# intel/hdk

Measured on AMD Instinct MI355X. Metric: rows/sec, 1B-row int64 GROUP BY SUM, higher is better.
Workload: dtype int64; 1 GPU; C2: SELECT key, SUM(val) GROUP BY key; int64, 64 uniform keys; rows=1000000000, rows_per_gpu=1000000000, fragments=32, fragments_per_gpu=32, fragment_rows=32000000, layout=perfect hash, keyless, 64 entries, parallelism=fragment f -> GPU f mod 1; one GPU

## Files before the change

hdk_amd/csrc/scan_bhm.hip:

```cpp
#include <string.h>

#include <algorithm>

#include "host_match.h"
#include "scan_bhm.h"
#include "scan_bhm_part.h"
#include "scan_bhm_host.h"
#include "scan_bhm_shapes.h"

namespace hdk {

constexpr uint32_t kBhmMaxLdsBytes = 144u << 10;
constexpr uint32_t kBhmSmallLdsBytes = 40u << 10;
constexpr uint32_t kBhmReplicatedBytes = 32u << 10;
constexpr int64_t kBhmMaxAbsVal = (1ll << 19) - 1;
static bool bhm_off() { return hdk_sw(SW_NO_BHM) != nullptr || hdk_sw(SW_NO_BH_LDS) != nullptr || hdk_sw(SW_NO_BH_DENSE) != nullptr; }

static uint32_t bits_for(uint64_t codes) {
  uint32_t b = 1;
  while ((1ull << b) < codes) ++b;
  return b;
}

struct BhmGeom {
// ... 269 lines not shown
      sw.packed = der.packed;
    } else if (sw.kind == BMW_NN) {
      if (!src.nullable) {
        sw.kind = BMW_ROWS;
        sw.packed = a->rows_packed;
      } else if (der.packed >= 0) {
        sw.packed = der.packed;
      } else {
        from_field(der.has_mx != 0);
      }
    } else {
      from_field(sw.kind == BMW_MAX);
    }
  }
  *per_entry_out = 8u * static_cast<uint32_t>(a->npacked) + static_cast<uint32_t>(a->mm_bytes) + (a->rows_packed < 0 ? 4u : 0u);
  *amax_out = amax;
  g->nk = a->nkeys;
  g->ns = a->nsrc;
  return true;
}

static uint64_t bhm_lds_layout(BhmArgs* a, uint32_t per_entry) {
  a->e1 = (a->entries + 1 + 1) & ~1u;
  a->off_mm = 8u * static_cast<uint32_t>(a->npacked) * a->e1;
  a->off_rows = a->off_mm + static_cast<uint32_t>(a->mm_bytes) * a->e1;
  return static_cast<uint64_t>(a->e1) * per_entry;
}

static bool match_bhm(const hdk_hip_plan* p, const hdk_hip_kernel_options* ko, BhmArgs* a, BhmGeom* g) {
  uint32_t per_entry;
  int64_t amax;
  if (!match_bhm_shape(p, ko, a, g, &per_entry, &amax)) return false;
  const uint64_t one = bhm_lds_layout(a, per_entry);
  if (one > kBhmMaxLdsBytes) return false;
  uint32_t rep_bytes = (static_cast<uint32_t>(one) + 15u) & ~15u;
  uint32_t rep = 16;
  while (rep > 1 && static_cast<uint64_t>(rep_bytes + 16) * rep > kBhmReplicatedBytes) rep >>= 1;
  if (rep > 1) {
    while (rep_bytes % 256 != 16) rep_bytes += 16;
  }
  a->rep = rep;
  a->rep_bytes = rep_bytes;
  a->lds_bytes = rep_bytes * rep;
  g->block = a->lds_bytes > kBhmSmallLdsBytes ? 1024 : 256;
  g->grid_per_cu = g->block == 1024 ? 1 : 3;
  const int64_t by_sum = ((1ll << 39) - 1) / amax;
  a->max_rows_per_block = static_cast<uint32_t>(std::min<int64_t>(by_sum, 1ll << 23));
  return true;
}

constexpr uint32_t kBhmPartLdsBytes = 50u << 10;
struct BhmPartLayout {
  size_t cursor_bytes, tuple_bytes, slab_bytes, total;
};
static bool match_bhm_part(const hdk_hip_plan* p, const hdk_hip_kernel_options* ko, BhmPartArgs* pg, BhmGeom* g, BhmPartLayout* l) {
  if (hdk_sw(SW_NO_BHM_PARTITIONS) || hdk_sw(SW_NO_BH_PARTITIONS)) return false;
  memset(pg, 0, sizeof(*pg));
  BhmArgs* a = &pg->b;
  uint32_t per_entry;
  int64_t amax;
  if (!match_bhm_shape(p, ko, a, g, &per_entry, &amax)) return false;
  const bool always = hdk_sw(SW_BH_PARTITIONS_ALWAYS) != nullptr;
  if (!always && ko->total_rows < (4ull << 20)) return false;
  const uint32_t total = a->entries;
  uint32_t w = 4;
  while (w < 14 && (static_cast<uint64_t>((2u << w) + 2) * per_entry) <= kBhmPartLdsBytes) ++w;
  uint32_t min_bins = 128;
  if (const char* e = hdk_sw(SW_BHM_PART_MIN_BINS)) min_bins = static_cast<uint32_t>(std::max(1, atoi(e)));
  while (w > 4 && ((total + (1u << w) - 1) >> w) < min_bins) --w;
  while (((total + (1u << w) - 1) >> w) > kPbMaxBins) ++w;
  if (static_cast<uint64_t>((1u << w) + 2) * per_entry > kBhmPartLdsBytes) return false;
  pg->w = w;
  pg->nbins = (total + (1u << w) - 1) >> w;
  pg->total_entries = total;
  uint32_t pos = w;
  for (int s = 0; s < a->nsrc; ++s) {
    const uint32_t cb = bits_for(static_cast<uint64_t>(a->src[s].raw_span) + 2);
    if (pos + cb > 32) return false;
    pg->cshift[s] = pos;
    pg->cmask[s] = static_cast<uint32_t>((1ull << cb) - 1);
    pos += cb;
  }
  pg->tw = (pos <= 16 && !hdk_sw(SW_BHM_WIDE_TUPLES)) ? 2 : 4;
  a->entries = 1u << w;
  const uint64_t one = bhm_lds_layout(a, per_entry);
  uint32_t prep_bytes = (static_cast<uint32_t>(one) + 15u) & ~15u;
  uint32_t prep = 1;
  if (const char* e = hdk_sw(SW_BHM_PART_REPLICAS)) prep = static_cast<uint32_t>(std::max(1, atoi(e)));
  while (prep > 1 && static_cast<uint64_t>(prep_bytes + 16) * prep > kBhmReplicatedBytes) prep >>= 1;
  if (prep > 1) {
    while (prep_bytes % 256 != 16) prep_bytes += 16;
  }
  a->rep = prep;
  a->rep_bytes = prep_bytes;
  a->lds_bytes = prep_bytes * prep;
  a->max_rows_per_block = 0xFFFFFFFFu;
  const int64_t by_sum = ((1ll << 39) - 1) / amax;
  uint64_t generation = static_cast<uint64_t>(std::min<int64_t>(by_sum, 1ll << 23)) & ~4095ull;
  if (const char* e = hdk_sw(SW_BHM_PART_GENERATION)) generation = static_cast<uint64_t>(std::max(1, atoi(e))) * 4096;
  if (generation < 4096) return false;
  pg->generation = static_cast<uint32_t>(generation);
  for (int w = 0; w < a->wpe; ++w) pg->wop[w] = g->wop[w];
  pg->cap_limit = 0xFFFFFFF0ull;
  pg->parts = 64;
  const uint64_t avg = ko->total_rows / (static_cast<uint64_t>(pg->nbins) * kPbXcds) + 1;
  pg->part_tuples = static_cast<uint32_t>(std::min<uint64_t>((std::max<uint64_t>(2 * avg, 65536) + 4095) & ~4095ull, 1u << 30));
  if (const char* e = hdk_sw(SW_BHM_PART_TUPLES)) pg->part_tuples = static_cast<uint32_t>(std::max(1, atoi(e))) * 4096u;
  pg->total_rows = ko->total_rows;
  pg->region_max = ((ko->total_rows / kPbXcds) * 5 / 2 + static_cast<uint64_t>(pg->nbins) * 4104 + 7) & ~7ull;
  if (pg->region_max > 0xFFFFFFF0ull) return false;
  pg->sample_stride = static_cast<uint32_t>(std::min<uint64_t>(std::max<uint64_t>(ko->total_rows / (256ull * (16 / g->width)) / 1536, 1), 1u << 16));
  if (const char* e = hdk_sw(SW_BHM_PART_SAMPLE_STRIDE)) pg->sample_stride = static_cast<uint32_t>(std::max(1, atoi(e)));
  l->cursor_bytes = static_cast<size_t>(pg->nbins) * kPbXcds * kPbCursorStride * sizeof(uint32_t) + kBlWords * sizeof(uint32_t);
  l->cursor_bytes = (l->cursor_bytes + 255) & ~static_cast<size_t>(255);
  l->tuple_bytes = std::max((static_cast<size_t>(kPbXcds) * pg->region_max + kBhmPartBlock * 16) * pg->tw, static_cast<size_t>(total) * a->wpe * 8);
  l->tuple_bytes = (l->tuple_bytes + 255) & ~static_cast<size_t>(255);
  l->slab_bytes = static_cast<size_t>(kPbXcds) * total * a->wpe * 8;
  if (l->slab_bytes > (1ull << 30)) return false;
  l->total = 256 + l->cursor_bytes + l->tuple_bytes + l->slab_bytes;
  return true;
}

HDK_BHM_DEFINE_KERNELS(4, false, HDK_BHM_SHAPE_FN_NULLS, HDK_BHM_PLAIN_BODY_YES)

struct BhmStaticShape {
  int nk, ns;
  uint32_t code[kBhmMaxDer];
  const void* (*aggregate)(int tw, bool nulls);
};
#define HDK_BHM_SHAPE_ROW(NK, NS, D0, D1, D2, D3)                                                                            \
  {NK, NS, {D0, D1, D2, D3}, [](int tw, bool nulls) -> const void* {                                                         \
     if (nulls) {                                                                                                            \
       return tw == 2 ? reinterpret_cast<const void*>(hdk_bhm_aggregate<BhmStatic<D0, D1, D2, D3, true>, NS, 2>)             \
                      : reinterpret_cast<const void*>(hdk_bhm_aggregate<BhmStatic<D0, D1, D2, D3, true>, NS, 4>);            \
     }                                                                                                                       \
     return tw == 2 ? reinterpret_cast<const void*>(hdk_bhm_aggregate<BhmStatic<D0, D1, D2, D3, false>, NS, 2>)              \
                    : reinterpret_cast<const void*>(hdk_bhm_aggregate<BhmStatic<D0, D1, D2, D3, false>, NS, 4>);             \
   }},
static const BhmStaticShape kBhmShapes[] = {HDK_BHM_SHAPES(HDK_BHM_SHAPE_ROW)};
#undef HDK_BHM_SHAPE_ROW
constexpr int kBhmNumShapes = static_cast<int>(sizeof(kBhmShapes) / sizeof(kBhmShapes[0]));

template <class F4, class F4Q, class F8, class F8Q>
static const void* bhm_by_quarter(const BhmArgs& a, const BhmGeom& g, F4 f4, F4Q f4q, F8 f8, F8Q f8q) {
  return g.width == 8 ? (a.nquals ? f8q() : f8()) : (a.nquals ? f4q() : f4());
}
static const void* bhm_scatter_kernel(const BhmArgs& a, const BhmGeom& g) {
  return bhm_by_quarter(
      a, g, [&] { return BhmKernels<4, false>::scatter(g.nk, g.ns); }, [&] { return BhmKernels<4, true>::scatter(g.nk, g.ns); },
      [&] { return BhmKernels<8, false>::scatter(g.nk, g.ns); }, [&] { return BhmKernels<8, true>::scatter(g.nk, g.ns); });
}

template <int W>
static const void* bhm_sample_kernel_w(int nk) {
  return nk == 1 ? reinterpret_cast<const void*>(hdk_bhm_part_sample<1, W>)
                 : (nk == 2 ? reinterpret_cast<const void*>(hdk_bhm_part_sample<2, W>) : reinterpret_cast<const void*>(hdk_bhm_part_sample<3, W>));
}
static const void* bhm_sample_kernel(const BhmGeom& g) { return g.width == 8 ? bhm_sample_kernel_w<8>(g.nk) : bhm_sample_kernel_w<4>(g.nk); }

static uint32_t bhm_plain_flags(const BhmArgs& a);
static void bhm_shift_to_codes(BhmArgs* a) {
  a->plain_flags = bhm_plain_flags(*a);
  for (int d = 0; d < a->nder; ++d) {
    BhmDer& der = a->der[d];
    const BhmSrc& src = a->src[der.src];
    if (der.mul == 1) {
// ... 75 lines not shown
      if (same) return sh.aggregate(tw, a.any_nullable != 0);
    }
  }
  if (bhm_plain_flags(a) && !hdk_sw(SW_BHM_DYNAMIC)) {
    return tw == 2 ? bhm_aggregate_plain<2>(g.ns) : bhm_aggregate_plain<4>(g.ns);
  }
  return tw == 2 ? bhm_aggregate_dynamic<2>(g.ns) : bhm_aggregate_dynamic<4>(g.ns);
}

const char* bhm_kernel_name(const hdk_hip_plan* p, const hdk_hip_kernel_options* ko) {
  BhmArgs a;
  BhmGeom g;
  if (!match_bhm(p, ko, &a, &g)) {
    BhmPartArgs pg;
    BhmPartLayout l;
    if (match_bhm_part(p, ko, &pg, &g, &l)) {
      return g.perfect ? "hdk_bhm_scatter,hdk_bhm_aggregate,hdk_bhm_reduce_slabs,hdk_finalize"
                       : "hdk_bhm_scatter,hdk_bhm_aggregate,hdk_bhm_reduce_slabs,hdk_bhm_fold";
    }
    return nullptr;
  }
  return g.perfect ? "hdk_scan_agg_bhm,hdk_bhm_reduce_slabs,hdk_finalize" : "hdk_scan_agg_bhm,hdk_bhm_reduce_slabs,hdk_bhm_fold";
}

static int32_t launch_bhm_folds(const hdk_hip_plan* plan, const hdk_hip_plan* d_plan, const KernParams& kp, const hdk_hip_kernel_options* ko,
                                const hdk_hip_device_properties* props, hipStream_t s, const BhmArgs& a, const BhmGeom& g, uint32_t entries,
                                const int64_t* fold_slabs, uint32_t fold_count) {
  int32_t st;
  if (g.perfect) {
    st = launch_finalize_slabs(d_plan, fold_slabs, kp.groupby_buf, fold_count, plan->entry_count, a.flag, s);
    if (st) return st;
  } else {
    BhmFoldArgs f;
    memset(&f, 0, sizeof(f));
    f.plan = d_plan;
    f.kp = kp;
    f.slabs = fold_slabs;
    f.flag = a.flag;
    f.num_slabs = fold_count;
    f.entries = entries;
    f.out_entry_count = plan->entry_count;
    f.wpe = a.wpe;
    for (int w = 0; w < a.wpe; ++w) f.wop[w] = g.wop[w];
    f.nword_mask = g.nword_mask;
    f.key_form = a.key_form;
    f.key_lo = g.key_lo;
    f.null_entry = g.null_entry;
    f.key_null_word = a.key_null_word;
    if (fold_count <= 16 && entries >= 2048) {
      hipLaunchKernelGGL(hdk_bhm_fold<1>, dim3((entries + 255) / 256), dim3(256), 0, s, f);
    } else {
      hipLaunchKernelGGL(hdk_bhm_fold<0>, dim3((entries + 3) / 4), dim3(256), 0, s, f);
    }
    HDK_HIP_CHECK(hipGetLastError());
  }
  if (hdk_sw(SW_BHM_FLAG_IS_ERROR)) {
    hipLaunchKernelGGL(hdk_bhm_flag_is_error<0>, dim3(1), dim3(1), 0, s, a.flag, kp.error_code);
    HDK_HIP_CHECK(hipGetLastError());
    return HDK_HIP_OK;
  }
  return launch_scan_global_armed(plan, d_plan, kp, ko, props, s, a.flag);
}

static int32_t launch_bhm_part(const hdk_hip_plan* plan, const hdk_hip_plan* d_plan, const KernParams& kp, const hdk_hip_kernel_options* ko,
                               const hdk_hip_device_properties* props, hipStream_t s, BhmPartArgs& pg, const BhmGeom& g, const BhmPartLayout& l,
                               bool* launched) {
  AsyncScratch scratch(s);
  if (hipMallocAsync(&scratch.p, l.total, s) != hipSuccess) {
    (void)hipGetLastError();
    scratch.p = nullptr;
    return HDK_HIP_OK;
  }
  int8_t* base = static_cast<int8_t*>(scratch.p);
  HDK_HIP_CHECK(hipMemsetAsync(base, 0, 256 + l.cursor_bytes, s));
  BhmArgs& a = pg.b;
  a.plan = d_plan;
  a.kp = kp;
  a.flag = reinterpret_cast<uint32_t*>(base);
  pg.fill = reinterpret_cast<uint32_t*>(base + 256);
  pg.layout = pg.fill + static_cast<size_t>(pg.nbins) * kPbXcds * kPbCursorStride;
  pg.tuples = reinterpret_cast<uint32_t*>(base + 256 + l.cursor_bytes);
  a.slabs = reinterpret_cast<int64_t*>(base + 256 + l.cursor_bytes + l.tuple_bytes);
  const void* sk = bhm_scatter_kernel(a, g);
  const size_t scatter_lds = bhm_scatter_lds(g.width);
  HDK_HIP_CHECK(hipFuncSetAttribute(sk, hipFuncAttributeMaxDynamicSharedMemorySize, static_cast<int>(scatter_lds)));
  const unsigned g1 = scatter_grid(sk, kBhmPartBlock, scatter_lds, props, kBhmPartWaves * 256 / kBhmPartBlock);
  void* kargs[] = {&pg};
  const uint64_t sampled_tiles = ko->total_rows / (256ull * (16 / g.width)) / pg.sample_stride + 1;
  const unsigned g0 = static_cast<unsigned>(std::min<uint64_t>((sampled_tiles + 3) / 4, static_cast<uint64_t>(props->num_cu)));
  HDK_HIP_CHECK(hipLaunchKernel(bhm_sample_kernel(g), dim3(g0), dim3(256), kargs, 0, s));
  HDK_HIP_CHECK(hipLaunchKernel(reinterpret_cast<const void*>(hdk_bhm_part_layout<0>), dim3(1), dim3(kPbMaxBins), kargs, 0, s));
  HDK_HIP_CHECK(hipLaunchKernel(sk, dim3(g1), dim3(kBhmPartBlock), kargs, scatter_lds, s));
  const void* ak = bhm_aggregate_kernel(a, g, static_cast<int>(pg.tw));
  BhmPartArgs pgb = pg;
  bhm_shift_to_codes(&pgb.b);
  void* kargs_b[] = {&pgb};
  if (a.lds_bytes > (48u << 10)) {
    HDK_HIP_CHECK(hipFuncSetAttribute(ak, hipFuncAttributeMaxDynamicSharedMemorySize, static_cast<int>(a.lds_bytes)));
  }
  {
    BhmSlabInitArgs ia;
    memset(&ia, 0, sizeof(ia));
    ia.slabs = a.slabs;
    ia.words = static_cast<uint64_t>(kPbXcds) * pg.total_entries * static_cast<uint32_t>(a.wpe);
    ia.wpe = a.wpe;
    for (int w = 0; w < a.wpe; ++w) ia.wop[w] = g.wop[w];
    const unsigned gi = static_cast<unsigned>(std::min<uint64_t>((ia.words + 255) / 256, static_cast<uint64_t>(props->num_cu) * 8));
    hipLaunchKernelGGL(hdk_bhm_slab_init<0>, dim3(gi), dim3(256), 0, s, ia);
    HDK_HIP_CHECK(hipGetLastError());
  }
  HDK_HIP_CHECK(hipLaunchKernel(ak, dim3(pg.nbins * kPbXcds, pg.parts), dim3(kBhmAggBlock), kargs_b, a.lds_bytes, s));
  BhmReduceArgs r;
  memset(&r, 0, sizeof(r));
  r.in = a.slabs;
  r.out = reinterpret_cast<int64_t*>(base + 256 + l.cursor_bytes);
  r.flag = a.flag;
  r.num_slabs = kPbXcds;
  r.groups = 1;
  r.words = pg.total_entries * static_cast<uint32_t>(a.wpe);
  r.wpe = a.wpe;
  for (int w = 0; w < a.wpe; ++w) r.wop[w] = g.wop[w];
  hipLaunchKernelGGL(hdk_bhm_reduce_slabs<0>, dim3((r.words + 255) / 256, 1), dim3(256), 0, s, r);
  HDK_HIP_CHECK(hipGetLastError());
  const int32_t st = launch_bhm_folds(plan, d_plan, kp, ko, props, s, a, g, pg.total_entries, r.out, 1);
  if (st) return st;
  *launched = true;
  return HDK_HIP_OK;
}

int32_t launch_bhm(const hdk_hip_plan* plan, const hdk_hip_plan* d_plan, const KernParams& kp, const hdk_hip_kernel_options* ko,
                   const hdk_hip_device_properties* props, hipStream_t s, bool* launched) {
  *launched = false;
  BhmArgs a;
  BhmGeom g;
  if (!match_bhm(plan, ko, &a, &g)) {
    BhmPartArgs pg;
    BhmPartLayout l;
    if (match_bhm_part(plan, ko, &pg, &g, &l)) return launch_bhm_part(plan, d_plan, kp, ko, props, s, pg, g, l, launched);
    return HDK_HIP_OK;
  }
  bool is_static;
  const void* k = bhm_kernel(a, g, &is_static);
  if (a.lds_bytes > (48u << 10)) {
    HDK_HIP_CHECK(hipFuncSetAttribute(k, hipFuncAttributeMaxDynamicSharedMemorySize, static_cast<int>(a.lds_bytes)));
  }
  const uint32_t cu = static_cast<uint32_t>(props->num_cu);
  uint32_t grid = std::min(resident_grid(k, g.block, a.lds_bytes, props), g.grid_per_cu * cu);
  if (const char* e = hdk_sw(SW_BHM_BLOCKS_PER_CU)) grid = std::max(1, atoi(e)) * cu;
  constexpr uint64_t kTileRows256 = 256ull * 4 * kBhmU;
  const uint64_t tile_rows = kTileRows256 * (g.block / 256);
  const uint64_t budget = a.max_rows_per_block > 4 * tile_rows ? a.max_rows_per_block - 4 * tile_rows : tile_rows;
  const uint64_t need = (2 * ko->total_rows + budget - 1) / budget;
  if (need > grid) grid = static_cast<uint32_t>(std::min<uint64_t>(need, 1u << 16));
  if (ko->grid_dim_x) grid = ko->grid_dim_x;
  const uint32_t words = a.entries * static_cast<uint32_t>(a.wpe);
  const uint32_t red_groups = grid > 16 ? 4u : 0u;
  const size_t slab_bytes = (static_cast<size_t>(grid) * words * 8 + 255) & ~static_cast<size_t>(255);
  const size_t red_bytes = static_cast<size_t>(red_groups) * words * 8;
  AsyncScratch scratch(s);
  if (hipMallocAsync(&scratch.p, 256 + slab_bytes + red_bytes, s) != hipSuccess) {
    (void)hipGetLastError();
    scratch.p = nullptr;
    return HDK_HIP_OK;
  }
  HDK_HIP_CHECK(hipMemsetAsync(scratch.p, 0, 256, s));
  a.plan = d_plan;
  a.kp = kp;
// ... 31 lines not shown
```

hdk_amd/csrc/scan_bhm_part.h:

```cpp
#pragma once
#include "scan_bhm.h"
#include "part_scatter_batch.h"

namespace hdk {

#ifndef HDK_BHM_PART_BLOCK
#define HDK_BHM_PART_BLOCK 512
#endif
constexpr int kBhmPartBlock = HDK_BHM_PART_BLOCK;
#ifndef HDK_BHM_PART_VR
#define HDK_BHM_PART_VR 16
#endif
#ifndef HDK_BHM_PART_WAVES
#define HDK_BHM_PART_WAVES 4
#endif
constexpr int kBhmPartWaves = HDK_BHM_PART_WAVES;
constexpr int bhm_part_vr(int w) { return w == 8 ? 8 : HDK_BHM_PART_VR; }
constexpr size_t bhm_scatter_lds(int w) { return static_cast<size_t>(kBhmPartBlock) * bhm_part_vr(w) * 8; }
constexpr int kBhmAggBlock = 256;

constexpr uint32_t kBlHist = 0;
constexpr uint32_t kBlSampled = 256;
constexpr uint32_t kBlCap = 512;
constexpr uint32_t kBlOff = 768;
constexpr uint32_t kBlRegion = 1024;
constexpr uint32_t kBlWords = 1032;

struct BhmPartArgs {
  BhmArgs b;
  uint32_t w;
  uint32_t nbins;
  uint32_t total_entries;
  uint32_t tw;
  uint32_t cshift[kBhmMaxSrc];
  uint32_t cmask[kBhmMaxSrc];
  uint64_t cap_limit;
  uint64_t region_max;
  uint64_t total_rows;
  uint32_t* tuples;
  uint32_t* fill;
  uint32_t* layout;
  uint32_t sample_stride;
  uint32_t parts;
  uint32_t part_tuples;
  uint32_t generation;
  int32_t wop[kMaxWordsPerEntry];
};

template <int NK, int W>
HDK_DEV uint32_t bhm_part_sample_bin(const BhmPartArgs& g, const uint32_t (&kr)[NK][4], int i, bool nulls) {
  const BhmArgs& a = g.b;
  uint32_t idx = 0;
#pragma unroll
  for (int kk = 0; kk < NK; ++kk) {
    const BhmKey& key = a.key[kk];
    bool wide;
    const int32_t kv = bhm_narrow<W>(kr[kk], i, wide);
    uint32_t d = min(static_cast<uint32_t>(kv) - static_cast<uint32_t>(key.min), key.n - 1u);
    if (nulls && key.nullable != 0 && kv == key.null32) {
      d = key.null_d;
    }
    idx += NK == 1 ? d : __umul24(d, key.stride);
  }
  return min(idx >> g.w, g.nbins - 1u);
}

template <int NK, int W>
__global__ __launch_bounds__(256) void hdk_bhm_part_sample(BhmPartArgs g) {
  constexpr int R = 16 / W;
  constexpr int64_t kTile = 256 * R;
  const BhmArgs& a = g.b;
  __shared__ uint32_t s_hist[kPbMaxBins];
  const int tid = threadIdx.x;
  s_hist[tid] = 0;
  __syncthreads();
  const uint64_t nfrag = *a.kp.num_fragments;
  const uint32_t ntab = *a.kp.num_tables;
  const bool nulls = a.any_nullable != 0;
  const int64_t stride = g.sample_stride;
  uint32_t seen = 0;
  int64_t tile = static_cast<int64_t>(blockIdx.x) * stride;
  int64_t frag_tile_begin = 0;
  for (uint64_t f = 0; f < nfrag; ++f) {
    const int64_t ntiles = a.kp.num_rows[f * ntab] / kTile;
    const int8_t* const* cols = a.kp.col_buffers[f];
    while (tile < frag_tile_begin + ntiles) {
      uint32_t kr[4][NK][4];
      bool have[4];
#pragma unroll
      for (int j = 0; j < 4; ++j) {
        const int64_t t = tile + j * static_cast<int64_t>(gridDim.x) * stride;
        have[j] = t < frag_tile_begin + ntiles;
        if (have[j]) {
          const int64_t r = (t - frag_tile_begin) * kTile + static_cast<int64_t>(tid) * R;
#pragma unroll
          for (int kk = 0; kk < NK; ++kk) {
            load_bytes<16, false>((gcol_t)cols[a.key[kk].buf_idx] + r * W, kr[j][kk]);
          }
        }
      }
#pragma unroll
      for (int j = 0; j < 4; ++j) {
        if (have[j]) {
#pragma unroll
          for (int i = 0; i < R; ++i) {
            atomicAdd(&s_hist[bhm_part_sample_bin<NK, W>(g, kr[j], i, nulls)], 1u);
          }
          seen += R;
          tile += static_cast<int64_t>(gridDim.x) * stride;
        }
      }
    }
    frag_tile_begin += ntiles;
  }
  __syncthreads();
  if (s_hist[tid]) {
// ... 76 lines not shown
      xv[s][i] = bhm_narrow<W>(xr[s], i, wide);
      if (W == 8) stale |= wide ? 1u : 0u;
    }
  }
  bool ok[R];
#pragma unroll
  for (int i = 0; i < R; ++i) {
    ok[i] = FULL || first_row + i < nrows;
  }
  if (Q) {
    if (qvec && a.qvec == 2) {
      const uint32_t lean = bhm_quals_lean<R, W, NK, NS>(a, kr, xr, qr);
#pragma unroll
      for (int i = 0; i < R; ++i) {
        ok[i] = ok[i] && ((lean >> i) & 1u) != 0;
      }
    } else if (qvec) {
      plain_quals_pass_with<R, true>(
          a.q, a.nquals,
          [&](int qi, const ProjFastQual&, const bool (&)[R], int64_t (&v)[R]) {
#pragma unroll
            for (int i = 0; i < R; ++i) {
              const int64_t v0 = extract_elem<W>(qr[0], i), v1 = extract_elem<W>(qr[1], i), v2 = extract_elem<W>(qr[2], i);
              v[i] = qi == 0 ? v0 : (qi == 1 ? v1 : v2);
            }
          },
          ok);
    } else {
      int64_t rows[R];
#pragma unroll
      for (int i = 0; i < R; ++i) {
        rows[i] = ok[i] ? first_row + i : 0;
      }
      plain_quals_pass<R, true>(a.q, a.nquals, cols, rows, ok, true);
    }
  }
#pragma unroll
  for (int i = 0; i < R; ++i) {
    uint32_t idx = 0;
#pragma unroll
    for (int kk = 0; kk < NK; ++kk) {
      const BhmKey& key = a.key[kk];
      uint32_t d = static_cast<uint32_t>(kv[kk][i]) - static_cast<uint32_t>(key.min);
      const bool isnull = NULLS && (key.nullable != 0) & (kv[kk][i] == key.null32);
      uint32_t seen = d;
      if (NULLS) {
        seen = isnull ? 0u : seen;
      }
      if (!FULL || Q) {
        seen = ok[i] ? seen : 0u;
      }
      kover[kk] = max(kover[kk], seen);
      d = min(d, key.n - 1u);
      if (NULLS) {
        d = isnull ? key.null_d : d;
      }
      idx += NK == 1 ? d : __umul24(d, key.stride);
    }
    uint32_t t = idx & wmask;
#pragma unroll
    for (int s = 0; s < NS; ++s) {
      const BhmSrc& src = a.src[s];
      uint32_t d = static_cast<uint32_t>(xv[s][i]) - static_cast<uint32_t>(src.raw_min);
      uint32_t code = d + 1u;
      if (NULLS) {
        const bool isnull = (src.nullable != 0) & (xv[s][i] == src.null32);
        d = isnull ? 0u : d;
        code = isnull ? 0u : code;
      }
      if (!FULL || Q) {
        d = ok[i] ? d : 0u;
      }
      sover[s] = max(sover[s], d);
      t |= code << g.cshift[s];
    }
    bin4[i] = (idx >> g.w) << 2;
    if (!FULL || Q) {
      bin4[i] = ok[i] ? bin4[i] : 4u * kPbMaxBins;
    }
    tup[i] = t;
  }
}

template <int NK, int NS, int W = 4, bool Q = false>
__global__ __launch_bounds__(kBhmPartBlock) __attribute__((amdgpu_waves_per_eu(kBhmPartWaves, kBhmPartWaves))) void hdk_bhm_scatter(BhmPartArgs g) {
  constexpr int VR = bhm_part_vr(W);
  constexpr int kBhmPartTile = kBhmPartBlock * VR;
  constexpr int R = 16 / W, U = VR / R;
  const BhmArgs& a = g.b;
  __shared__ uint32_t s_cnt[kPbMaxBins + 1];
  __shared__ uint2 s_pair[kPbMaxBins + 1];
  __shared__ int32_t s_watch;
  extern __shared__ __attribute__((aligned(16))) uint32_t s_dyn32[];
  const int tid = threadIdx.x;
  const uint32_t xcd = static_cast<uint32_t>(__builtin_amdgcn_s_getreg(20 | (0 << 6) | (3 << 11))) & (kPbXcds - 1);
  for (int i = tid; i <= kPbMaxBins; i += kBhmPartBlock) {
    s_cnt[i] = 0;
  }
  const uint64_t region = (static_cast<uint64_t>(g.layout[kBlRegion + 1]) << 32) | g.layout[kBlRegion];
  uint8_t* const xcd_tuples = reinterpret_cast<uint8_t*>(g.tuples) + static_cast<size_t>(xcd) * region * g.tw;
  uint32_t my_cap = 0, my_off = 0;
  if (tid < kPbMaxBins) {
    my_cap = g.layout[kBlCap + tid];
    my_off = g.layout[kBlOff + tid];
  }
  __syncthreads();
  const uint64_t nfrag = *a.kp.num_fragments;
  const uint32_t ntab = *a.kp.num_tables;
  int32_t err = 0;
  uint32_t stale = 0;
  uint32_t kover[NK], sover[NS];
#pragma unroll
  for (int kk = 0; kk < NK; ++kk) {
    kover[kk] = 0;
  }
#pragma unroll
  for (int s = 0; s < NS; ++s) {
    sover[s] = 0;
  }
  const Watch watch = watch_begin(a.kp);
  const bool nulls = a.any_nullable != 0;
  const bool narrow = g.tw == 2;
  int64_t tile = blockIdx.x;
  int64_t frag_tile_begin = 0;
  bool stop = false;
  for (uint64_t f = 0; f < nfrag && !stop; ++f) {
    const int64_t nrows = a.kp.num_rows[f * ntab];
    const int64_t ntiles = (nrows + kBhmPartTile - 1) / kBhmPartTile;
    const int8_t* const* cols = a.kp.col_buffers[f];
    gcol_t kcol[NK], xcol[NS];
#pragma unroll
    for (int kk = 0; kk < NK; ++kk) {
      kcol[kk] = (gcol_t)cols[a.key[kk].buf_idx];
    }
#pragma unroll
    for (int s = 0; s < NS; ++s) {
      xcol[s] = (gcol_t)cols[a.src[s].buf_idx];
    }
    for (; tile < frag_tile_begin + ntiles; tile += gridDim.x) {
      if (watch.flags) {
        if (const int32_t wv = watch_poll_block(watch, &s_watch)) {
          err = wv;
          stop = true;
          break;
        }
      }
      const int64_t row0 = (tile - frag_tile_begin) * kBhmPartTile;
      const bool full = row0 + kBhmPartTile <= nrows;
      uint32_t tup[VR], bin4[VR];
      uint32_t kr[U][NK][4], xr[U][NS][4], qr[Q ? U : 1][kMaxPlainQuals][4];
      const bool qvec = Q && full && a.qvec != 0;
#define HDK_BHM_PART_LOAD(ROW0)                                                                       \
  _Pragma("unroll") for (int u = 0; u < U; ++u) {                                                    \
    const int64_t r = (ROW0) + (static_cast<int64_t>(u) * kBhmPartBlock + tid) * R;                       \
    _Pragma("unroll") for (int kk = 0; kk < NK; ++kk) {                                              \
      load_bytes<16, true>(kcol[kk] + r * W, kr[u][kk]);                                             \
    }                                                                                                \
    _Pragma("unroll") for (int s = 0; s < NS; ++s) {                                                 \
      load_bytes<16, true>(xcol[s] + r * W, xr[u][s]);                                               \
    }                                                                                                \
    _Pragma("unroll") for (int qi = 0; qi < kMaxPlainQuals; ++qi) {                                  \
      if (Q && a.qvec != 0 && qi < a.nquals && (a.qvec != 2 || a.qsrc[qi] == kBhmQualOwnLoad)) {     \
        load_bytes<16, true>((gcol_t)cols[a.q[qi].col.buf_idx] + r * W, qr[Q ? u : 0][qi]);          \
      }                                                                                              \
    }                                                                                                \
  }
      if (full) {
        HDK_BHM_PART_LOAD(row0)
      } else {
#pragma unroll
        for (int u = 0; u < U; ++u) {
#pragma unroll
          for (int i = 0; i < R; ++i) {
            const int64_t r = row0 + (static_cast<int64_t>(u) * kBhmPartBlock + tid) * R + i;
            const bool in = r < nrows;
#pragma unroll
            for (int kk = 0; kk < NK; ++kk) {
              const int64_t v = in ? load_elem<W>(kcol[kk], r) : 0;
              if (W == 8) {
                kr[u][kk][(2 * i) % 4] = static_cast<uint32_t>(v);
                kr[u][kk][(2 * i + 1) % 4] = static_cast<uint32_t>(static_cast<uint64_t>(v) >> 32);
              } else {
                kr[u][kk][i % 4] = static_cast<uint32_t>(v);
              }
            }
#pragma unroll
            for (int s = 0; s < NS; ++s) {
              const int64_t v = in ? load_elem<W>(xcol[s], r) : 0;
              if (W == 8) {
                xr[u][s][(2 * i) % 4] = static_cast<uint32_t>(v);
                xr[u][s][(2 * i + 1) % 4] = static_cast<uint32_t>(static_cast<uint64_t>(v) >> 32);
              } else {
                xr[u][s][i % 4] = static_cast<uint32_t>(v);
              }
            }
          }
        }
      }
#define HDK_BHM_PART_ROWS(FULL_, NULLS_)                                                                                          \
  _Pragma("unroll") for (int u = 0; u < U; ++u) {                                                                                \
    bhm_part_rows<NK, NS, W, Q, FULL_, NULLS_>(g, cols, kr[u], xr[u], qr[Q ? u : 0], qvec,                                       \
                                               row0 + (static_cast<int64_t>(u) * kBhmPartBlock + tid) * (16 / W), nrows, &tup[u * (16 / W)], \
                                               &bin4[u * (16 / W)], kover, sover, stale);                                        \
  }
      if (full) {
        if (nulls) {
          HDK_BHM_PART_ROWS(true, true)
        } else {
          HDK_BHM_PART_ROWS(true, false)
        }
      } else if (nulls) {
        HDK_BHM_PART_ROWS(false, true)
      } else {
        HDK_BHM_PART_ROWS(false, false)
      }
#undef HDK_BHM_PART_ROWS
#undef HDK_BHM_PART_LOAD
      uint32_t rank[VR];
#pragma unroll
      for (int r = 0; r < VR; ++r) {
        rank[r] = (!Q || bin4[r] != 4u * kPbMaxBins) ? atomicAdd(reinterpret_cast<uint32_t*>(reinterpret_cast<uint8_t*>(s_cnt) + bin4[r]), 1u) : 0u;
      }
      __syncthreads();
      if (tid < kPbMaxBins) {
        const uint32_t n = s_cnt[tid];
        uint32_t base = 0;
        if (n) {
          base = atomicAdd(g.fill + (static_cast<size_t>(xcd) * g.nbins + tid) * kPbCursorStride, n);
        }
        const int lane = tid & (kWave - 1), wv = tid / kWave;
        uint32_t incl = n;
#pragma unroll
        for (int dd = 1; dd < kWave; dd <<= 1) {
          const uint32_t v = __shfl_up(incl, dd, kWave);
          if (lane >= dd) {
            incl += v;
          }
        }
        uint32_t before = 0;
        for (int c = 0; c < wv; ++c) {
          uint32_t v = s_cnt[c * kWave + lane];
#pragma unroll
          for (int dd = kWave / 2; dd >= 1; dd >>= 1) {
            v += __shfl_xor(v, dd, kWave);
          }
          before += v;
        }
        const uint32_t x = before + incl - n;
        if (n && static_cast<uint64_t>(base) + n > my_cap) {
          stale = 1;
          base = min(base, my_cap);
        }
        s_pair[tid] = make_uint2(x, my_off + base);
        if (tid == kPbMaxBins - 1) {
          s_pair[kPbMaxBins] = make_uint2(x + n, 0u);
        }
      }
      __syncthreads();
      uint2* const stage = reinterpret_cast<uint2*>(s_dyn32);
#pragma unroll
      for (int r = 0; r < VR; ++r) {
        if (!Q || bin4[r] != 4u * kPbMaxBins) {
          const uint2 pr = *reinterpret_cast<const uint2*>(reinterpret_cast<const uint8_t*>(s_pair) + 2u * bin4[r]);
          stage[pr.x + rank[r]] = make_uint2(tup[r], pr.y + rank[r]);
        }
      }
      if (tid < kPbMaxBins) {
        s_cnt[tid] = 0;
      }
      if (tid == 0) {
        s_cnt[kPbMaxBins] = 0;
      }
      __syncthreads();
      const uint32_t total = s_pair[kPbMaxBins].x;
      if (narrow) {
        for (uint32_t i = tid; i < total; i += kBhmPartBlock) {
          const uint2 v = stage[i];
          reinterpret_cast<uint16_t*>(xcd_tuples)[v.y] = static_cast<uint16_t>(v.x);
        }
      } else {
        for (uint32_t i = tid; i < total; i += kBhmPartBlock) {
          const uint2 v = stage[i];
          reinterpret_cast<uint32_t*>(xcd_tuples)[v.y] = v.x;
        }
      }
    }
    frag_tile_begin += ntiles;
  }
#pragma unroll
  for (int kk = 0; kk < NK; ++kk) {
    stale |= kover[kk] >= a.key[kk].n ? 1u : 0u;
  }
#pragma unroll
  for (int s = 0; s < NS; ++s) {
    stale |= sover[s] > a.src[s].raw_span ? 1u : 0u;
  }
  if (stale) {
    atomicOr(a.flag, 1u);
  }
  if (err) {
    record_error(a.kp.error_code, err);
  }
}

struct BhmSlabInitArgs {
  int64_t* slabs;
  uint64_t words;
  int32_t wpe;
  int32_t wop[kMaxWordsPerEntry];
};
template <int DUMMY = 0>
__global__ __launch_bounds__(256) void hdk_bhm_slab_init(BhmSlabInitArgs a) {
  for (uint64_t i = static_cast<uint64_t>(blockIdx.x) * 256 + threadIdx.x; i < a.words; i += static_cast<uint64_t>(gridDim.x) * 256) {
    a.slabs[i] = word_identity(a.wop[i % static_cast<uint32_t>(a.wpe)]);
  }
}

template <class C, int NS, int TW = 4>
__global__ __launch_bounds__(kBhmAggBlock) void hdk_bhm_aggregate(BhmPartArgs g) {
  const BhmArgs& a = g.b;
  extern __shared__ __attribute__((aligned(16))) uint8_t lds8[];
  const int tid = threadIdx.x;
  if (*a.flag) {
    return;
  }
  const uint32_t bin = blockIdx.x / kPbXcds, x = blockIdx.x % kPbXcds;
  const size_t sub = static_cast<size_t>(x) * g.nbins + bin;
  const uint32_t n_sub = min(g.fill[sub * kPbCursorStride], g.layout[kBlCap + bin]);
  const uint32_t nparts = n_sub > 2 * static_cast<uint64_t>(g.part_tuples) ? min(g.parts, (n_sub + g.part_tuples - 1) / g.part_tuples) : 1u;
  if (blockIdx.y >= max(nparts, 1u)) {
    return;
  }
  const bool shared = nparts > 1;
  uint32_t part_begin = 0, n = n_sub;
  if (shared) {
    const uint32_t chunk = (((n_sub + nparts - 1) / nparts) + 4095u) & ~4095u;
    part_begin = min(blockIdx.y * chunk, n_sub);
    n = min(part_begin + chunk, n_sub) - part_begin;
  }
  {
    uint4* z = reinterpret_cast<uint4*>(lds8);
    const uint32_t n16 = a.lds_bytes / 16;
    for (uint32_t i = tid; i < n16; i += kBhmAggBlock) {
      z[i] = make_uint4(0, 0, 0, 0);
    }
  }
  __syncthreads();
  uint8_t* rp = lds8 + static_cast<size_t>(tid & (a.rep - 1)) * a.rep_bytes;
  const uint64_t region = (static_cast<uint64_t>(g.layout[kBlRegion + 1]) << 32) | g.layout[kBlRegion];
  const uint8_t* t = reinterpret_cast<const uint8_t*>(g.tuples) + (static_cast<size_t>(x) * region + g.layout[kBlOff + bin] + part_begin) * TW;
  const uint32_t wmask = (1u << g.w) - 1u;
  const uint32_t dummy = a.entries;
  const bool nulls = C::nulls(a);
  constexpr int TPV = 16 / TW;
  constexpr int U = 16 / TPV;
  constexpr int R = 4;
  constexpr uint32_t kStep = kBhmAggBlock * TPV * U;
  typedef uint32_t __attribute__((ext_vector_type(4))) u32x4_t;
#define HDK_BHM_AGG_ROWS(FULL_)                                                                                  \
  _Pragma("unroll") for (int u = 0; u < U; ++u) {                                                               \
    const uint32_t i = base + (static_cast<uint32_t>(u) * kBhmAggBlock + tid) * TPV;                            \
    const uint32_t wd[4] = {tv[u].x, tv[u].y, tv[u].z, tv[u].w};                                                \
    _Pragma("unroll") for (int h = 0; h < TPV / R; ++h) {                                                       \
      uint32_t e[R];                                                                                            \
      int32_t xv[NS][R];                                                                                        \
      bool lv[NS][R];                                                                                           \
      _Pragma("unroll") for (int j = 0; j < R; ++j) {                                                           \
        const int jj = h * R + j;                                                                               \
        const uint32_t tup = TW == 2 ? (wd[jj / 2] >> (16 * (jj & 1))) & 0xFFFFu : wd[jj % 4];                  \
        const bool in = FULL_ || (i + jj < n);                                                                  \
        e[j] = in ? tup & wmask : dummy;                                                                        \
        _Pragma("unroll") for (int s = 0; s < NS; ++s) {                                                        \
          const uint32_t code = (tup >> g.cshift[s]) & g.cmask[s];                                              \
          xv[s][j] = static_cast<int32_t>(code);                                                                \
          lv[s][j] = nulls ? (in & (code != 0)) : true;                                                         \
        }                                                                                                       \
      }                                                                                                         \
      bhm_update<C, NS, R, false>(a, rp, dummy, e, xv, lv);                                               \
    }                                                                                                           \
  }
  const uint32_t e0 = bin << g.w;
  int64_t* slab = a.slabs + static_cast<size_t>(x) * g.total_entries * a.wpe;
  bool flushed = false;
  auto flush = [&]() {
// ... 81 lines not shown
```

Before: 426.3 billion rows/s.

## Pack bin index into staged tuples and shrink scatter register and LDS footprint

The scatter kernel now packs each row's rank above its bin offset in a single register and stages one 32-bit word per row instead of a uint2. The bin is embedded in the tuple's high bits, or kept in a side byte array, and the destination is rebuilt from a per-bin delta table. Scatter LDS drops from 8 to 4 or 5 bytes per row. Other changes cut register pressure: uniform values go through readfirstlane, kernel arguments are reloaded from the kernarg pointer, and addressing uses 32-bit offsets. The partial-tile path is also simplified with clamped loads, at the cost of more intricate bit packing and the static limits it depends on.

```diff
diff --git a/hdk_amd/csrc/scan_bhm.hip b/hdk_amd/csrc/scan_bhm.hip
--- a/hdk_amd/csrc/scan_bhm.hip
+++ b/hdk_amd/csrc/scan_bhm.hip
@@ -375,6 +375,8 @@
     pos += cb;
   }
   pg->tw = (pos <= 16 && !hdk_sw(SW_BHM_WIDE_TUPLES)) ? 2 : 4;
+  pg->bshift = pos + 9 <= 32 ? pos : 0;
+  pg->tmask = pos >= 32 ? 0xFFFFFFFFu : (1u << pos) - 1u;
   a->entries = 1u << w;
   const uint64_t one = bhm_lds_layout(a, per_entry);
   uint32_t prep_bytes = (static_cast<uint32_t>(one) + 15u) & ~15u;
@@ -616,7 +618,7 @@
   pg.tuples = reinterpret_cast<uint32_t*>(base + 256 + l.cursor_bytes);
   a.slabs = reinterpret_cast<int64_t*>(base + 256 + l.cursor_bytes + l.tuple_bytes);
   const void* sk = bhm_scatter_kernel(a, g);
-  const size_t scatter_lds = bhm_scatter_lds(g.width);
+  const size_t scatter_lds = bhm_scatter_lds(g.width, pg.bshift != 0);
   HDK_HIP_CHECK(hipFuncSetAttribute(sk, hipFuncAttributeMaxDynamicSharedMemorySize, static_cast<int>(scatter_lds)));
   const unsigned g1 = scatter_grid(sk, kBhmPartBlock, scatter_lds, props, kBhmPartWaves * 256 / kBhmPartBlock);
   void* kargs[] = {&pg};
diff --git a/hdk_amd/csrc/scan_bhm_part.h b/hdk_amd/csrc/scan_bhm_part.h
--- a/hdk_amd/csrc/scan_bhm_part.h
+++ b/hdk_amd/csrc/scan_bhm_part.h
@@ -16,7 +16,9 @@
 #endif
 constexpr int kBhmPartWaves = HDK_BHM_PART_WAVES;
 constexpr int bhm_part_vr(int w) { return w == 8 ? 8 : HDK_BHM_PART_VR; }
-constexpr size_t bhm_scatter_lds(int w) { return static_cast<size_t>(kBhmPartBlock) * bhm_part_vr(w) * 8; }
+constexpr size_t bhm_scatter_lds(int w, bool packed) {
+  return static_cast<size_t>(kBhmPartBlock) * bhm_part_vr(w) * (packed ? 4 : 5);
+}
 constexpr int kBhmAggBlock = 256;
 
 constexpr uint32_t kBlHist = 0;
@@ -32,6 +34,8 @@
   uint32_t nbins;
   uint32_t total_entries;
   uint32_t tw;
+  uint32_t bshift;
+  uint32_t tmask;
   uint32_t cshift[kBhmMaxSrc];
   uint32_t cmask[kBhmMaxSrc];
   uint64_t cap_limit;
@@ -274,16 +278,35 @@
   }
 }
 
+HDK_DEV uint64_t bhm_uniform64(uint64_t v) {
+  const uint32_t lo = __builtin_amdgcn_readfirstlane(static_cast<uint32_t>(v));
+  const uint32_t hi = __builtin_amdgcn_readfirstlane(static_cast<uint32_t>(v >> 32));
+  return (static_cast<uint64_t>(hi) << 32) | lo;
+}
+typedef const __attribute__((address_space(4))) BhmPartArgs* bhm_kernarg_t;
+HDK_DEV bhm_kernarg_t bhm_args_again() {
+  auto p = __builtin_amdgcn_kernarg_segment_ptr();
+  asm volatile("" : "+s"(p));
+  return (bhm_kernarg_t)p;
+}
+constexpr uint32_t kBhmRankShift = 11;
+constexpr uint32_t kBhmBin4Mask = (1u << kBhmRankShift) - 1u;
+
 template <int NK, int NS, int W = 4, bool Q = false>
 __global__ __launch_bounds__(kBhmPartBlock) __attribute__((amdgpu_waves_per_eu(kBhmPartWaves, kBhmPartWaves))) void hdk_bhm_scatter(BhmPartArgs g) {
   constexpr int VR = bhm_part_vr(W);
   constexpr int kBhmPartTile = kBhmPartBlock * VR;
   constexpr int R = 16 / W, U = VR / R;
+  static_assert(kBhmPartTile <= (1 << (32 - kBhmRankShift)) && kBhmPartTile <= 8192, "a rank rides above its bin's offset");
   const BhmArgs& a = g.b;
   __shared__ uint32_t s_cnt[kPbMaxBins + 1];
-  __shared__ uint2 s_pair[kPbMaxBins + 1];
+  __shared__ uint32_t s_start[kPbMaxBins + 1];
+  __shared__ uint32_t s_delta[kPbMaxBins];
+  __shared__ uint2 s_sub[kPbMaxBins];
   __shared__ int32_t s_watch;
   extern __shared__ __attribute__((aligned(16))) uint32_t s_dyn32[];
+  uint32_t* const stage = s_dyn32;
+  uint8_t* const s_binof = reinterpret_cast<uint8_t*>(s_dyn32 + kBhmPartTile);
   const int tid = threadIdx.x;
   const uint32_t xcd = static_cast<uint32_t>(__builtin_amdgcn_s_getreg(20 | (0 << 6) | (3 << 11))) & (kPbXcds - 1);
   for (int i = tid; i <= kPbMaxBins; i += kBhmPartBlock) {
@@ -291,14 +314,12 @@
   }
   const uint64_t region = (static_cast<uint64_t>(g.layout[kBlRegion + 1]) << 32) | g.layout[kBlRegion];
   uint8_t* const xcd_tuples = reinterpret_cast<uint8_t*>(g.tuples) + static_cast<size_t>(xcd) * region * g.tw;
-  uint32_t my_cap = 0, my_off = 0;
   if (tid < kPbMaxBins) {
-    my_cap = g.layout[kBlCap + tid];
-    my_off = g.layout[kBlOff + tid];
+    s_sub[tid] = make_uint2(g.layout[kBlCap + tid], g.layout[kBlOff + tid]);
   }
   __syncthreads();
-  const uint64_t nfrag = *a.kp.num_fragments;
-  const uint32_t ntab = *a.kp.num_tables;
+  const uint32_t nfrag = __builtin_amdgcn_readfirstlane(static_cast<uint32_t>(*a.kp.num_fragments));
+  const uint32_t ntab = __builtin_amdgcn_readfirstlane(*a.kp.num_tables);
   int32_t err = 0;
   uint32_t stale = 0;
   uint32_t kover[NK], sover[NS];
@@ -310,90 +331,114 @@
   for (int s = 0; s < NS; ++s) {
     sover[s] = 0;
   }
-  const Watch watch = watch_begin(a.kp);
+  const uint32_t watch_flags = __builtin_amdgcn_readfirstlane(a.kp.watch->flags);
   const bool nulls = a.any_nullable != 0;
-  const bool narrow = g.tw == 2;
-  int64_t tile = blockIdx.x;
-  int64_t frag_tile_begin = 0;
+  uint32_t tile = blockIdx.x;
+  uint32_t frag_tile_begin = 0;
   bool stop = false;
-  for (uint64_t f = 0; f < nfrag && !stop; ++f) {
-    const int64_t nrows = a.kp.num_rows[f * ntab];
-    const int64_t ntiles = (nrows + kBhmPartTile - 1) / kBhmPartTile;
-    const int8_t* const* cols = a.kp.col_buffers[f];
-    gcol_t kcol[NK], xcol[NS];
+  for (uint32_t f = 0; f < nfrag && !stop; ++f) {
+    const int64_t nrows = static_cast<int64_t>(bhm_uniform64(static_cast<uint64_t>(a.kp.num_rows[static_cast<uint64_t>(f) * ntab])));
+    const uint32_t ntiles = static_cast<uint32_t>((nrows + kBhmPartTile - 1) / kBhmPartTile);
+    const int8_t* const* cols = reinterpret_cast<const int8_t* const*>(bhm_uniform64(reinterpret_cast<uintptr_t>(a.kp.col_buffers[f])));
+    gcol_t kfrag[NK], xfrag[NS];
 #pragma unroll
     for (int kk = 0; kk < NK; ++kk) {
-      kcol[kk] = (gcol_t)cols[a.key[kk].buf_idx];
+      kfrag[kk] = (gcol_t)bhm_uniform64(reinterpret_cast<uintptr_t>(cols[a.key[kk].buf_idx]));
     }
 #pragma unroll
     for (int s = 0; s < NS; ++s) {
-      xcol[s] = (gcol_t)cols[a.src[s].buf_idx];
+      xfrag[s] = (gcol_t)bhm_uniform64(reinterpret_cast<uintptr_t>(cols[a.src[s].buf_idx]));
     }
     for (; tile < frag_tile_begin + ntiles; tile += gridDim.x) {
-      if (watch.flags) {
-        if (const int32_t wv = watch_poll_block(watch, &s_watch)) {
+      if (watch_flags) {
+        if (const int32_t wv = watch_poll_block(watch_begin(a.kp), &s_watch)) {
           err = wv;
           stop = true;
           break;
         }
       }
-      const int64_t row0 = (tile - frag_tile_begin) * kBhmPartTile;
+      int bt = tid;
+      asm volatile("" : "+v"(bt));
+      const int64_t row0 = static_cast<int64_t>(tile - frag_tile_begin) * kBhmPartTile;
       const bool full = row0 + kBhmPartTile <= nrows;
-      uint32_t tup[VR], bin4[VR];
+      const uint32_t rem = full ? static_cast<uint32_t>(kBhmPartTile) : static_cast<uint32_t>(nrows - row0);
+      gcol_t kcol[NK], xcol[NS];
+#pragma unroll
+      for (int kk = 0; kk < NK; ++kk) {
+        kcol[kk] = kfrag[kk] + row0 * W;
+      }
+#pragma unroll
+      for (int s = 0; s < NS; ++s) {
+        xcol[s] = xfrag[s] + row0 * W;
+      }
+      uint32_t tup[VR], br[VR];
       uint32_t kr[U][NK][4], xr[U][NS][4], qr[Q ? U : 1][kMaxPlainQuals][4];
       const bool qvec = Q && full && a.qvec != 0;
-#define HDK_BHM_PART_LOAD(ROW0)                                                                       \
-  _Pragma("unroll") for (int u = 0; u < U; ++u) {                                                    \
-    const int64_t r = (ROW0) + (static_cast<int64_t>(u) * kBhmPartBlock + tid) * R;                       \
+#define HDK_BHM_PART_LOAD_STEP(u)                                                                     \
+  {                                                                                                  \
+    uint32_t voff = (static_cast<uint32_t>(u) * kBhmPartBlock + bt) * 16u;                           \
+        \
+        \
+    asm volatile("" : "+v"(voff));                                                                   \
     _Pragma("unroll") for (int kk = 0; kk < NK; ++kk) {                                              \
-      load_bytes<16, true>(kcol[kk] + r * W, kr[u][kk]);                                             \
+      load_bytes<16, true>(kcol[kk] + voff, kr[u][kk]);                                              \
     }                                                                                                \
     _Pragma("unroll") for (int s = 0; s < NS; ++s) {                                                 \
-      load_bytes<16, true>(xcol[s] + r * W, xr[u][s]);                                               \
+      load_bytes<16, true>(xcol[s] + voff, xr[u][s]);                                                \
     }                                                                                                \
-    _Pragma("unroll") for (int qi = 0; qi < kMaxPlainQuals; ++qi) {                                  \
-      if (Q && a.qvec != 0 && qi < a.nquals && (a.qvec != 2 || a.qsrc[qi] == kBhmQualOwnLoad)) {     \
-        load_bytes<16, true>((gcol_t)cols[a.q[qi].col.buf_idx] + r * W, qr[Q ? u : 0][qi]);          \
-      }                                                                                              \
-    }                                                                                                \
   }
       if (full) {
-        HDK_BHM_PART_LOAD(row0)
+#pragma unroll
+        for (int u = 0; u < U; ++u) {
+          HDK_BHM_PART_LOAD_STEP(u)
+#pragma unroll
+          for (int qi = 0; qi < kMaxPlainQuals; ++qi) {
+            if (Q && a.qvec != 0 && qi < a.nquals && (a.qvec != 2 || a.qsrc[qi] == kBhmQualOwnLoad)) {
+              const int64_t r = row0 + (static_cast<int64_t>(u) * kBhmPartBlock + bt) * R;
+              load_bytes<16, true>((gcol_t)cols[a.q[qi].col.buf_idx] + r * W, qr[Q ? u : 0][qi]);
+            }
+          }
+        }
       } else {
 #pragma unroll
         for (int u = 0; u < U; ++u) {
-#pragma unroll
-          for (int i = 0; i < R; ++i) {
-            const int64_t r = row0 + (static_cast<int64_t>(u) * kBhmPartBlock + tid) * R + i;
-            const bool in = r < nrows;
-#pragma unroll
-            for (int kk = 0; kk < NK; ++kk) {
-              const int64_t v = in ? load_elem<W>(kcol[kk], r) : 0;
-              if (W == 8) {
-                kr[u][kk][(2 * i) % 4] = static_cast<uint32_t>(v);
-                kr[u][kk][(2 * i + 1) % 4] = static_cast<uint32_t>(static_cast<uint64_t>(v) >> 32);
-              } else {
-                kr[u][kk][i % 4] = static_cast<uint32_t>(v);
+          const uint32_t lr = (static_cast<uint32_t>(u) * kBhmPartBlock + bt) * R;
+          if (lr + R <= rem) {
+            HDK_BHM_PART_LOAD_STEP(u)
+          } else {
+#pragma unroll
+            for (int i = 0; i < R; ++i) {
+              const uint32_t er = min(lr + i, rem - 1u);
+#pragma unroll
+              for (int kk = 0; kk < NK; ++kk) {
+                const int64_t v = load_elem<W>(kcol[kk] + er * static_cast<uint32_t>(W), 0);
+                if (W == 8) {
+                  kr[u][kk][(2 * i) % 4] = static_cast<uint32_t>(v);
+                  kr[u][kk][(2 * i + 1) % 4] = static_cast<uint32_t>(static_cast<uint64_t>(v) >> 32);
+                } else {
+                  kr[u][kk][i % 4] = static_cast<uint32_t>(v);
+                }
+              }
+#pragma unroll
+              for (int s = 0; s < NS; ++s) {
+                const int64_t v = load_elem<W>(xcol[s] + er * static_cast<uint32_t>(W), 0);
+                if (W == 8) {
+                  xr[u][s][(2 * i) % 4] = static_cast<uint32_t>(v);
+                  xr[u][s][(2 * i + 1) % 4] = static_cast<uint32_t>(static_cast<uint64_t>(v) >> 32);
+                } else {
+                  xr[u][s][i % 4] = static_cast<uint32_t>(v);
+                }
               }
             }
-#pragma unroll
-            for (int s = 0; s < NS; ++s) {
-              const int64_t v = in ? load_elem<W>(xcol[s], r) : 0;
-              if (W == 8) {
-                xr[u][s][(2 * i) % 4] = static_cast<uint32_t>(v);
-                xr[u][s][(2 * i + 1) % 4] = static_cast<uint32_t>(static_cast<uint64_t>(v) >> 32);
-              } else {
-                xr[u][s][i % 4] = static_cast<uint32_t>(v);
-              }
-            }
-          }
-        }
-      }
+          }
+        }
+      }
+#undef HDK_BHM_PART_LOAD_STEP
 #define HDK_BHM_PART_ROWS(FULL_, NULLS_)                                                                                          \
   _Pragma("unroll") for (int u = 0; u < U; ++u) {                                                                                \
     bhm_part_rows<NK, NS, W, Q, FULL_, NULLS_>(g, cols, kr[u], xr[u], qr[Q ? u : 0], qvec,                                       \
-                                               row0 + (static_cast<int64_t>(u) * kBhmPartBlock + tid) * (16 / W), nrows, &tup[u * (16 / W)], \
-                                               &bin4[u * (16 / W)], kover, sover, stale);                                        \
+                                               row0 + (static_cast<int64_t>(u) * kBhmPartBlock + bt) * (16 / W), nrows, &tup[u * (16 / W)], \
+                                               &br[u * (16 / W)], kover, sover, stale);                                          \
   }
       if (full) {
         if (nulls) {
@@ -401,26 +446,25 @@
         } else {
           HDK_BHM_PART_ROWS(true, false)
         }
-      } else if (nulls) {
+      } else {
         HDK_BHM_PART_ROWS(false, true)
-      } else {
-        HDK_BHM_PART_ROWS(false, false)
       }
 #undef HDK_BHM_PART_ROWS
-#undef HDK_BHM_PART_LOAD
-      uint32_t rank[VR];
+      const bhm_kernarg_t ga = bhm_args_again();
 #pragma unroll
       for (int r = 0; r < VR; ++r) {
-        rank[r] = (!Q || bin4[r] != 4u * kPbMaxBins) ? atomicAdd(reinterpret_cast<uint32_t*>(reinterpret_cast<uint8_t*>(s_cnt) + bin4[r]), 1u) : 0u;
+        const uint32_t rank = (!Q || br[r] != 4u * kPbMaxBins) ? atomicAdd(reinterpret_cast<uint32_t*>(reinterpret_cast<uint8_t*>(s_cnt) + br[r]), 1u) : 0u;
+        br[r] |= rank << kBhmRankShift;
       }
       __syncthreads();
-      if (tid < kPbMaxBins) {
-        const uint32_t n = s_cnt[tid];
+      if (bt < kPbMaxBins) {
+        const uint32_t n = s_cnt[bt];
+        const uint32_t my_cap = s_sub[bt].x, my_off = s_sub[bt].y;
         uint32_t base = 0;
         if (n) {
-          base = atomicAdd(g.fill + (static_cast<size_t>(xcd) * g.nbins + tid) * kPbCursorStride, n);
-        }
-        const int lane = tid & (kWave - 1), wv = tid / kWave;
+          base = atomicAdd(ga->fill + (xcd * ga->nbins + static_cast<uint32_t>(bt)) * kPbCursorStride, n);
+        }
+        const int lane = bt & (kWave - 1), wv = bt / kWave;
         uint32_t incl = n;
 #pragma unroll
         for (int dd = 1; dd < kWave; dd <<= 1) {
@@ -443,55 +487,75 @@
           stale = 1;
           base = min(base, my_cap);
         }
-        s_pair[tid] = make_uint2(x, my_off + base);
-        if (tid == kPbMaxBins - 1) {
-          s_pair[kPbMaxBins] = make_uint2(x + n, 0u);
+        s_start[bt] = x;
+        s_delta[bt] = my_off + base - x;
+        if (bt == kPbMaxBins - 1) {
+          s_start[kPbMaxBins] = x + n;
         }
       }
       __syncthreads();
-      uint2* const stage = reinterpret_cast<uint2*>(s_dyn32);
+      const uint32_t bshift = ga->bshift;
 #pragma unroll
       for (int r = 0; r < VR; ++r) {
-        if (!Q || bin4[r] != 4u * kPbMaxBins) {
-          const uint2 pr = *reinterpret_cast<const uint2*>(reinterpret_cast<const uint8_t*>(s_pair) + 2u * bin4[r]);
-          stage[pr.x + rank[r]] = make_uint2(tup[r], pr.y + rank[r]);
-        }
-      }
-      if (tid < kPbMaxBins) {
-        s_cnt[tid] = 0;
-      }
-      if (tid == 0) {
-        s_cnt[kPbMaxBins] = 0;
+        br[r] += *reinterpret_cast<const uint32_t*>(reinterpret_cast<const uint8_t*>(s_start) + (br[r] & kBhmBin4Mask)) << kBhmRankShift;
+      }
+      if (bshift) {
+        const uint32_t tmask = ga->tmask;
+#pragma unroll
+        for (int r = 0; r < VR; ++r) {
+          const uint32_t bin4 = br[r] & kBhmBin4Mask;
+          if (!Q || bin4 != 4u * kPbMaxBins) {
+            stage[br[r] >> kBhmRankShift] = (tup[r] & tmask) | (bin4 << (bshift - 2u));
+          }
+        }
+      } else {
+#pragma unroll
+        for (int r = 0; r < VR; ++r) {
+          const uint32_t bin4 = br[r] & kBhmBin4Mask;
+          if (!Q || bin4 != 4u * kPbMaxBins) {
+            stage[br[r] >> kBhmRankShift] = tup[r];
+            s_binof[br[r] >> kBhmRankShift] = static_cast<uint8_t>(bin4 >> 2);
+          }
+        }
+      }
+      if (bt <= kPbMaxBins) {
+        s_cnt[bt] = 0;
       }
       __syncthreads();
-      const uint32_t total = s_pair[kPbMaxBins].x;
-      if (narrow) {
-        for (uint32_t i = tid; i < total; i += kBhmPartBlock) {
-          const uint2 v = stage[i];
-          reinterpret_cast<uint16_t*>(xcd_tuples)[v.y] = static_cast<uint16_t>(v.x);
+      const uint32_t total = s_start[kPbMaxBins];
+      if (ga->tw == 2) {
+        for (uint32_t i = bt; i < total; i += kBhmPartBlock) {
+          const uint32_t v = stage[i];
+          reinterpret_cast<uint16_t*>(xcd_tuples)[s_delta[v >> bshift] + i] = static_cast<uint16_t>(v);
+        }
+      } else if (bshift) {
+        const uint32_t tmask = ga->tmask;
+        for (uint32_t i = bt; i < total; i += kBhmPartBlock) {
+          const uint32_t v = stage[i];
+          reinterpret_cast<uint32_t*>(xcd_tuples)[s_delta[v >> bshift] + i] = v & tmask;
         }
       } else {
-        for (uint32_t i = tid; i < total; i += kBhmPartBlock) {
-          const uint2 v = stage[i];
-          reinterpret_cast<uint32_t*>(xcd_tuples)[v.y] = v.x;
+        for (uint32_t i = bt; i < total; i += kBhmPartBlock) {
+          reinterpret_cast<uint32_t*>(xcd_tuples)[s_delta[s_binof[i]] + i] = stage[i];
         }
       }
     }
     frag_tile_begin += ntiles;
   }
+  const bhm_kernarg_t ge = bhm_args_again();
 #pragma unroll
   for (int kk = 0; kk < NK; ++kk) {
-    stale |= kover[kk] >= a.key[kk].n ? 1u : 0u;
+    stale |= kover[kk] >= ge->b.key[kk].n ? 1u : 0u;
   }
 #pragma unroll
   for (int s = 0; s < NS; ++s) {
-    stale |= sover[s] > a.src[s].raw_span ? 1u : 0u;
+    stale |= sover[s] > ge->b.src[s].raw_span ? 1u : 0u;
   }
   if (stale) {
-    atomicOr(a.flag, 1u);
+    atomicOr(ge->b.flag, 1u);
   }
   if (err) {
-    record_error(a.kp.error_code, err);
+    record_error(ge->b.kp.error_code, err);
   }
 }
 
```

New measurement: 426.0 billion rows/s. Within noise of the previous version (-0.1%).
